# ZHENGXi-git/TC-VIML

Hardware: AMD Instinct MI355X
Metric: sliding-window solves/sec (10 kf, 200 pt, 40 line) (higher is better)
Workload: dtype f64; 1 GPU; configs[2]: synthetic 10-kf window, 200 point + 40 2D-3D line residual blocks + marginalisation prior (n=75), 50 landmarks; 8 fixed dogleg iterations + 1 MARGIN_OLD marginalisation per solve; windows_per_gpu=1024, parallelism=independent windows x1, threads_per_window=256, layout=chain

## Files before the change

### tc-viml_amd/csrc/tcv_marg.hip

```cpp
#include <hip/hip_runtime.h>

#include "tcv_factors.h"
#include "tcv_marg.h"
#include "tcv_dev.h"

namespace tcv {

__device__ __forceinline__ int pidx(int a, int b) { return a >= b ? a * (a + 1) / 2 + b : b * (b + 1) / 2 + a; }


__device__ __forceinline__ void jacobi_angle(double app, double aqq, double apq, double tiny, double &c, double &s, bool &rot) {
    c = 1.0; s = 0.0; rot = false;
    if (fabs(apq) > tiny && fabs(apq) > 1e-15 * sqrt(fabs(app) * fabs(aqq))) {
        const double tau = (aqq - app) / (2.0 * apq);
        const double t = (tau >= 0 ? 1.0 : -1.0) / (fabs(tau) + sqrt(1.0 + tau * tau));
        c = 1.0 / sqrt(1.0 + t * t);
        s = t * c;
        rot = true;
    }
}
template <int MARG_NT, typename VP>
__device__ __noinline__ int jacobi_eig(lds_d *M, VP *V, int d, int ld, lds_d *rot, lds_i *cnt, int tid, double floor_rel, gbl_d *prof = nullptr) {
    long long t_last = clock64();
#ifdef TCV_PROFILE
// ... 611 lines not shown
            for (int i = n - 2; i > rbest; i--) {
                dm = fma(-e2[i], fast_rcp(dm), dv[i] - l);
                if (fabs(dm) < pivmin) dm = -pivmin;
                Z[i * ld + k] = dm;
            }
        }
        double z = 1.0, nrm2 = 1.0;
        for (int i = rbest - 1; i >= 0; i--) {
            z = -ev[i] * fast_rcp(Z[i * ld + k]) * z;
            Z[i * ld + k] = z;
            nrm2 += z * z;
        }
        z = 1.0;
        for (int i = rbest; i + 1 < n; i++) {
            z = -ev[i] * fast_rcp(Z[(i + 1) * ld + k]) * z;
            Z[(i + 1) * ld + k] = z;
            nrm2 += z * z;
        }
        Z[rbest * ld + k] = 1.0;
        const double sc = 1.0 / sqrt(nrm2);
        for (int i = 0; i < n; i++) Z[i * ld + k] *= sc;
        resid = gbest * sc;
    }
    __syncthreads();
    EMARK(2);
    if (wave == 0) {
        const double ctol = 1e-10 * tnorm;
        int start = -1;
        for (int k = 0; k < n; k++) {
            if (!(lam[k] > 1e-8)) continue;
            if (start < 0 || lam[k] - lam[k - 1] > ctol || !(lam[k - 1] > 1e-8)) { start = k; continue; }
            for (int pass = 0; pass < 2; pass++)
                for (int j = start; j < k; j++) {
                    double dot = 0;
                    for (int r = lane; r < n; r += 64) dot += Z[r * ld + j] * Z[r * ld + k];
                    for (int o = 32; o > 0; o >>= 1) dot += __shfl_xor(dot, o);
                    for (int r = lane; r < n; r += 64) Z[r * ld + k] -= dot * Z[r * ld + j];
                    __builtin_amdgcn_fence(__ATOMIC_ACQ_REL, "wavefront");
                }
            double nn = 0;
            for (int r = lane; r < n; r += 64) { const double t = Z[r * ld + k]; nn += t * t; }
            for (int o = 32; o > 0; o >>= 1) nn += __shfl_xor(nn, o);
            const double sc = 1.0 / sqrt(nn);
            for (int r = lane; r < n; r += 64) Z[r * ld + k] *= sc;
            __builtin_amdgcn_fence(__ATOMIC_ACQ_REL, "wavefront");
        }
    }
    __syncthreads();
    EMARK(3);
    {
        int c0 = 0;
        if (!old_search) { while (c0 < n && !(lam[c0] > 1e-8)) c0++; }
        if (!(flags & 2)) eig_backtransform_wy<NT>(Hq, Z, tauv, vbuf, n, ld, tid, c0);
        else if (NT >= 512 || n - c0 <= 16 * NW) eig_backtransform<4>(Hq, Z, tauv, n, ld, tid, c0);
        else eig_backtransform<3>(Hq, Z, tauv, n, ld, tid, c0);
    }
    __syncthreads();
    EMARK(4);
    double dev = 0;
    {
        lds_d *u1 = vbuf, *u2 = pbuf;
        if (tid < n) {
            double a1 = 0, a2 = 0;
            for (int k = 0; k < n; k++) if (lam[k] > 1e-8) { const double zz = Z[tid * ld + k]; a1 += zz; a2 += (k & 1) ? -zz : zz; }
            u1[tid] = a1; u2[tid] = a2;
        }
        __syncthreads();
        if (tid < n && lam[tid] > 1e-8) {
            double t1 = 0, t2 = 0;
            for (int r2 = 0; r2 < n; r2++) { const double zz = Z[r2 * ld + tid]; t1 += zz * u1[r2]; t2 += zz * u2[r2]; }
            dev = fmax(fabs(t1 - 1.0), fabs(t2 - ((tid & 1) ? -1.0 : 1.0)));
        }
    }
    for (int o = 32; o > 0; o >>= 1) { dev = fmax(dev, __shfl_xor(dev, o)); resid = fmax(resid, __shfl_xor(resid, o)); }
    __syncthreads();
    if (lane == 0) { red[wave] = dev; red[8 + wave] = resid; }
    __syncthreads();
    dev = 0; resid = 0;
#pragma unroll
    for (int w = 0; w < NW; w++) { dev = fmax(dev, red[w]); resid = fmax(resid, red[8 + w]); }
    double sl = 0;
    for (int i = 0; i < n; i++) sl += lam[i];
    __syncthreads();
    EMARK(5);
    if (tid == 0 && dbg) { dbg[0] = dev; dbg[1] = sl; dbg[2] = trace; dbg[3] = tnorm; dbg[4] = lam[0]; dbg[5] = lam[n - 1]; }
    if (!old_search) return (dev < 1e-7) && (resid <= 1e-9 * fmax(tnorm, 1e-300) * n) && (dev == dev) && (resid == resid);
    return (dev < 1e-7) && (fabs(sl - trace) <= 1e-9 * fmax(tnorm, 1e-300) * n) && (dev == dev);
}

#ifdef TCV_PROFILE
#define MARG_MARK(id) do { const long long t_ = clock64(); if (tid == 0) out[MARG_DIAG_PHASE + (id)] += (double)(t_ - t_last); t_last = t_; } while (0)
#define MARG_SUB(id) do { const long long t_ = clock64(); if (tid == 0) out[MARG_DIAG_PROJ_SUB + (id)] += (double)(t_ - t_sub); t_sub = t_; } while (0)
#else
#define MARG_MARK(id) do { } while (0)
#define MARG_SUB(id) do { } while (0)
#endif
template <int MREG>
__device__ __noinline__ void chol_small_regs(lds_d *Mm_, lds_d *okflag_, int m_, int ldm_, int tid) {
    lds_d *Mm = opaque_lds(Mm_), *okflag = opaque_lds(okflag_);
    const int m = uni_i<2>(m_), ldm = uni_i<2>(ldm_);
    if (tid < 64) {
        const int i = min(tid, m - 1);
        double t[MREG];
#pragma unroll
        for (int c = 0; c < MREG; c++) { const double a = pin_f64(Mm[i * ldm + min(c, m - 1)]); t[c] = c < m ? a : 0.0; }
        bool ok = true;
#pragma unroll
        for (int k = 0; k < MREG; k++) {
            const double sd = lane_f64(t[k], k);
            ok = ok && (k >= m || ((sd > 0.0) && (sd < 1e300)));
            const double rs = 1.0 / sqrt((ok && k < m) ? sd : 1.0);
            const double lik = t[k] * rs;
#pragma unroll
            for (int c = k + 1; c < MREG; c++) t[c] -= lik * lane_f64(lik, c);
            if (tid < m && tid > k) Mm[tid * ldm + k] = lik;
            if (tid == k && k < m) Mm[k * ldm + k] = rs;
        }
        if (tid == 0) *okflag = ok ? 1.0 : 0.0;
    }
}
template <int MREG>
__device__ __noinline__ void fwd_small_regs(const lds_d *Mm_, const lds_d *Apk_, const lds_d *bv_, lds_d *Zl_, lds_d *rot_, int m_, int n_, int ldm_, int zs_, int tid) {
    const lds_d *Mm = opaque_lds(Mm_), *Apk = opaque_lds(Apk_), *bv = opaque_lds(bv_);
    lds_d *Zl = opaque_lds(Zl_), *rot = opaque_lds(rot_);
    const int m = uni_i<2>(m_), n = uni_i<2>(n_), ldm = uni_i<2>(ldm_), zs = uni_i<2>(zs_);
    if (tid < n + 1 + m) {
        const int j = tid, ju = tid - n - 1;
        double z[MREG];
#pragma unroll
        for (int k = 0; k < MREG; k++) {
            const int kc = min(k, m - 1);
            const double a = pin_f64(Apk[pidx(m + min(j, n - 1), kc)]), bb = pin_f64(bv[kc]);
            z[k] = k < m ? (j < n ? a : (j == n ? bb : (k == ju ? 1.0 : 0.0))) : 0.0;
        }
        double nn = 0.0;
#pragma unroll
        for (int k = 0; k < MREG; k++) {
            const int kc = min(k, m - 1);
            double l[MREG];
            const double lkk = Mm[kc * ldm + kc];
#pragma unroll
            for (int k2 = k + 1; k2 < MREG; k2++) l[k2] = Mm[min(k2, m - 1) * ldm + kc];
            z[k] *= lkk;
            nn = (k >= ju && k < m) ? fma(z[k], z[k], nn) : nn;
#pragma unroll
            for (int k2 = k + 1; k2 < MREG; k2++) z[k2] = pin_f64(z[k2] - l[k2] * z[k]);
            if (j <= n && k < m) Zl[k * zs + j] = z[k];
            __builtin_amdgcn_sched_barrier(0);
        }
        if (j > n) rot[ju] = nn;
    }
}

#ifndef TCV_MARG_WAVES
#define TCV_MARG_WAVES 2
#endif
template <int MARG_NT>
__global__ void __launch_bounds__(MARG_NT) __attribute__((disable_tail_calls)) __attribute__((amdgpu_waves_per_eu(TCV_MARG_WAVES, TCV_MARG_WAVES))) marg_kernel(MargArgs Aarg) {
    extern __shared__ __attribute__((aligned(16))) double lds_raw[];
    lds_d *lds = (lds_d *)lds_raw;
    const int tid = threadIdx.x;
    gbl_d *scr = (gbl_d *)Aarg.scratch + (size_t)blockIdx.x * MARG_SCR_STRIDE;
    for (int win = blockIdx.x; win < Aarg.nwin; win += gridDim.x) {
        typedef const __attribute__((address_space(4))) MargHdr cst_mh;
        cst_mh &H = ((cst_mh *)Aarg.hdr)[win];
        cst_i *ip = (cst_i *)Aarg.ipool + H.ibase;
        cst_d *dp = (cst_d *)Aarg.dpool + H.dbase;
        const int pos = H.pos, m = H.m, n = H.n;
        if (H.nblk == 0) {
            if (tid == 0) { ((gbl_i *)Aarg.out_status)[win] = 0; ((gbl_i *)Aarg.out_status)[Aarg.nwin + win] = 0; }
            continue;
        }
        const int npk = pos * (pos + 1) / 2;
        lds_d *Apk = lds;
        const int me = m + (m & 1), ne = n + (n & 1);
        const int r1 = max(npk, ne * (ne + 1));
        lds_d *R2 = lds + ((r1 + 1) & ~1);
        const int cb_in_r2 = (H.cb_off >= 0 && H.cb_off >= ((r1 + 1) & ~1)) ? MARG_CB_LM * H.cb_stride + 2 * MARG_CB_LM : 0;
        const int r2 = max(max((int)MARG_STAGE + cb_in_r2, me * (me + 1) + max(me * (me + 1), m * (n + 1))), (n - 2) * (n - 1) / 2 + 1);
        lds_d *bv = R2 + ((r2 + 1) & ~1);
        lds_d *x = bv + MARG_MAX_POS;
        lds_d *rot = x + ((H.nx + 7) & ~7);
        lds_d *lam = rot + 160;
        lds_d *cvec = lam + MARG_MAX_N;
        lds_d *lmacc = cvec + MARG_MAX_POS;
        lds_d *sm = lmacc + 8;
        lds_d *stage = R2;
        lds_i *cnt = (lds_i *)(rot + 158);
        gbl_d *out = (gbl_d *)Aarg.out + (size_t)win * MARG_OUT_STRIDE;
        long long t_last = clock64();
        if (tid == 0) for (int i = 0; i < 12; i++) out[MARG_DIAG_PHASE + i] = 0.0;

        cst_i *blk = ip + H.o_blk;
        for (int b = tid; b < H.nblk; b += MARG_NT) {
            const int gs = blk[b * 5], go = blk[b * 5 + 1], xs = blk[b * 5 + 4];
            for (int i = 0; i < gs; i++)
                x[go + i] = (Aarg.use_solved_state && xs >= 0 && Aarg.solve_state)
                                ? ((const gbl_d *)Aarg.solve_state)[(size_t)H.solve_window * Aarg.state_stride + xs + i]
                                : dp[H.d_x + go + i];
        }
        for (int i = tid; i < pos; i += MARG_NT) { bv[i] = 0.0; cvec[i] = 0.0; }
        if (tid < 8) lmacc[tid] = 0.0;
        cst_d *misc = dp + H.d_misc;
        const double G3[3] = {misc[0], misc[1], misc[2]};
        __syncthreads();

        MARG_MARK(0);
        bool a_zeroed = false;
        if (H.prior_n > 0) {
            const int np = H.prior_n, k0 = H.prior_k0 >= 0 ? H.prior_k0 : ((cst_win *)Aarg.solve_win)[H.solve_window].prior_k0, nr = np - k0;
            cst_d *J0 = H.prior_abs >= 0 ? (cst_d *)Aarg.solve_dpool + H.prior_abs : dp + H.d_prior, *r0 = J0 + nr * np, *x0 = r0 + nr;
            lds_d *pdx = sm, *pr = sm + 128;
            if (tid < H.prior_nblk) {
                cst_i *pb = ip + H.o_prior + tid * 4;
                const int gs = pb[2], ls = gs == 7 ? 6 : gs;
                double x0v[16], xv[16], dxv[16];
                for (int i = 0; i < 16; i++) { x0v[i] = (i < gs) ? x0[pb[3] + i] : 0.0; xv[i] = (i < gs) ? x[blk[pb[0] * 5 + 1] + i] : 0.0; }
                prior_block_dx(xv, x0v, gs, dxv);
                for (int i = 0; i < 16; i++) if (i < ls) pdx[pb[1] + i] = dxv[i];
            }
            cst_i *pcol = ip + H.o_pcol;
            const bool in_lds = np <= MARG_MAX_N && nr * np <= r1;
            lds_d *Js = Apk;
            if (in_lds) {
                for (int e = tid; e < nr * np; e += 4 * MARG_NT) {
                    double v4[4];
#pragma unroll
                    for (int k = 0; k < 4; k++) if (e + k * MARG_NT < nr * np) v4[k] = J0[e + k * MARG_NT];
#pragma unroll
                    for (int k = 0; k < 4; k++) if (e + k * MARG_NT < nr * np) Js[e + k * MARG_NT] = v4[k];
                }
            } else {
                for (int i = tid; i < npk; i += MARG_NT) Apk[i] = 0.0;
                a_zeroed = true;
            }
            __syncthreads();
            if (tid < nr) {
                double r = r0[tid];
                if (in_lds) {
                    int j = 0;
                    for (; j + 3 < np; j += 4) {
                        double a4[4], d4[4];
#pragma unroll
                        for (int u = 0; u < 4; u++) { a4[u] = Js[tid + nr * (j + u)]; d4[u] = pdx[j + u]; }
#pragma unroll
                        for (int u = 0; u < 4; u++) r += a4[u] * d4[u];
                    }
                    for (; j < np; j++) r += Js[tid + nr * j] * pdx[j];
                }
                else for (int j = 0; j < np; j++) r += J0[tid + nr * j] * pdx[j];
                pr[tid] = r;
            }
            __syncthreads();
            if (in_lds) {
                typedef double v4f64 __attribute__((ext_vector_type(4)));
                constexpr int NWV = MARG_NT / 64;
                const int nt16 = (np + 15) >> 4, lane = tid & 63, wave = tid >> 6;
                const int m16 = lane & 15, k4 = lane >> 4;
                v4f64 accs[4];
#pragma unroll
                for (int slot = 0; slot < 4; slot++) {
                    const int t = wave + slot * NWV;
                    v4f64 acc = {0.0, 0.0, 0.0, 0.0};
                    if (t < nt16 * (nt16 + 1) / 2) {
                        int ta = 0;
                        while ((ta + 1) * (ta + 2) / 2 <= t) ta++;
                        const int tb = t - ta * (ta + 1) / 2;
                        const int a = 16 * ta + m16, b = 16 * tb + m16;
                        const lds_d *ca = Js + nr * min(a, np - 1), *cb = Js + nr * min(b, np - 1);
                        for (int i0 = k0 & ~15; i0 < np; i0 += 16) {
                            double av[4], bv4[4];
#pragma unroll
                            for (int u = 0; u < 4; u++) {
                                const int i = i0 + 4 * u + k4, ic = max(0, min(i, np - 1) - k0);
                                const double xa = ca[ic], y = cb[ic];
                                av[u] = (i >= k0 && i < np && a < np) ? xa : 0.0; bv4[u] = (i >= k0 && i < np && b < np) ? y : 0.0;
                            }
#pragma unroll
                            for (int u = 0; u < 4; u++) acc = __builtin_amdgcn_mfma_f64_16x16x4f64(av[u], bv4[u], acc, 0, 0, 0);
                        }
                    }
                    accs[slot] = acc;
                }
                double s2 = 0;
                const bool mine = tid < np && pcol[min(tid, np - 1)] >= 0;
                if (mine) {
                    int i = 0;
                    for (; i + 3 < nr; i += 4) {
                        double a4[4], r4[4];
#pragma unroll
                        for (int u = 0; u < 4; u++) { a4[u] = Js[i + u + nr * tid]; r4[u] = pr[i + u]; }
#pragma unroll
                        for (int u = 0; u < 4; u++) s2 += a4[u] * r4[u];
                    }
                    for (; i < nr; i++) s2 += Js[i + nr * tid] * pr[i];
                }
                __syncthreads();
                for (int i = tid; i < npk; i += MARG_NT) Apk[i] = 0.0;
                a_zeroed = true;
                __syncthreads();
#pragma unroll
                for (int slot = 0; slot < 4; slot++) {
                    const int t = wave + slot * NWV;
                    if (t < nt16 * (nt16 + 1) / 2) {
                        int ta = 0;
                        while ((ta + 1) * (ta + 2) / 2 <= t) ta++;
                        const int tb = t - ta * (ta + 1) / 2;
#pragma unroll
                        for (int i = 0; i < 4; i++) {
                            const int ga = 16 * ta + 4 * i + k4, gb = 16 * tb + m16;
                            if (ga < np && gb <= ga) { const int ia = pcol[ga], ib = pcol[gb]; if (ia >= 0 && ib >= 0) Apk[pidx(ia, ib)] += accs[slot][i]; }
                        }
                    }
                }
                if (mine) bv[pcol[tid]] += s2;
            } else {
                for (int e = tid; e < np * np; e += MARG_NT) {
                    const int a = e / np, b = e - a * np;
                    if (b > a) continue;
                    const int ia = pcol[a], ib = pcol[b];
                    if (ia < 0 || ib < 0) continue;
                    double s0 = 0;
                    for (int i = 0; i < nr; i++) s0 += J0[i + nr * a] * J0[i + nr * b];
                    Apk[pidx(ia, ib)] += s0;
                }
                if (tid < np && pcol[tid] >= 0) {
                    double s2 = 0;
                    for (int i = 0; i < nr; i++) s2 += J0[i + nr * tid] * pr[i];
                    bv[pcol[tid]] += s2;
                }
            }
            __syncthreads();
        }
        if (!a_zeroed) {
            for (int i = tid; i < npk; i += MARG_NT) Apk[i] = 0.0;
            __syncthreads();
        }
        MARG_MARK(1);
        cst_d *imu0 = H.imu_abs >= 0 ? (cst_d *)Aarg.solve_dpool + H.imu_abs : dp + H.d_imu;
        for (int f = 0; f < H.n_imu; f++) {
            cst_i *b = ip + H.o_imu + f * 4;
            lds_d *S = stage + 1500;
            const bool s_given = Aarg.solve_sqrt != nullptr && H.sqrt_src >= 0 && H.n_imu == 1;
            if (s_given) { for (int i = tid; i < 225; i += MARG_NT) S[i] = ((const gbl_d *)Aarg.solve_sqrt)[(size_t)H.solve_window * 225 + i]; }
            else if (tid < 16) (void)imu_sqrt_info_group(imu0 + f * IMU_CONST + IMU_COV, S, stage + 512, stage + 512 + 225, tid);
            constexpr int RW0 = MARG_NT >= 320 ? 1 : 0, RLANE = MARG_NT >= 320 ? 0 : 32;
            if ((tid & 63) == RLANE && (tid >> 6) >= RW0 && (tid >> 6) < RW0 + 4) {
                double cst[62];
#pragma unroll
                for (int i = 0; i < 62; i++) cst[i] = imu0[f * IMU_CONST + i];
                imu_raw_part((tid >> 6) - RW0, CGEN(x + blk[b[0] * 5 + 1]), CGEN(x + blk[b[1] * 5 + 1]), CGEN(x + blk[b[2] * 5 + 1]),
                             CGEN(x + blk[b[3] * 5 + 1]), cst, G3, GEN(stage), IMU_STRIDE_J, true);
            }
            __syncthreads();
            if (tid < 31) {
                lds_d *rec = stage + tid;
                double v[15];
                for (int r = 0; r < 15; r++) v[r] = rec[r * IMU_STRIDE_J];
                for (int r = 0; r < 15; r++) {
                    double a = 0;
                    for (int s2 = r; s2 < 15; s2++) a += S[r * 15 + s2] * v[s2];
                    rec[r * IMU_STRIDE_J] = a;
                }
            }
            __syncthreads();
            const int colc[4] = {0, 6, 15, 21};
            for (int e = tid; e < 30 * 31; e += MARG_NT) {
                const int ca = e / 31, cb = e - ca * 31;
                if (cb < 30 && cb > ca) continue;
                int sa = 0, sb = 0;
                while (sa < 3 && ca >= colc[sa + 1]) sa++;
                const int la = blk[b[sa] * 5 + 2];
                if (la < 0) continue;
                const int ia = la + ca - colc[sa];
                double s = 0;
                for (int r = 0; r < 15; r++) s += stage[r * IMU_STRIDE_J + ca] * stage[r * IMU_STRIDE_J + cb];
                if (cb == 30) { bv[ia] += s; continue; }
                while (sb < 3 && cb >= colc[sb + 1]) sb++;
                const int lb = blk[b[sb] * 5 + 2];
                if (lb < 0) continue;
                Apk[pidx(ia, lb + cb - colc[sb])] += s;
            }
            __syncthreads();
        }
        MARG_MARK(2);
        const bool with_td = H.td_blk >= 0;
        const int prs = with_td ? 21 : (int)PROJ_STRIDE, prr = with_td ? 43 : (int)PROJ_REC;
        const int njc = with_td ? 20 : 19;
        const bool cb_path = H.block_mode && H.cb_off >= 0;
#ifdef TCV_PROFILE
        long long t_sub = clock64();
        if (tid == 0) for (int i = 0; i < 4; i++) out[MARG_DIAG_PROJ_SUB + i] = 0.0;
#endif
        MARG_SUB(0);
        typedef __attribute__((address_space(3))) unsigned char lds_b;
        lds_i *gtab = (lds_i *)sm, *ncls = gtab + 336;
        lds_b *listS = (lds_b *)(gtab + 340), *listJ = listS + 96, *listL = listJ + 104;
        if (cb_path) {
            if (tid < 3) ncls[tid] = 0;
            __syncthreads();
            const int ntri = 19 * 20 / 2;
            if (tid < ntri + 19) {
                int ca, cb;
                if (tid < ntri) { ca = (int)((sqrt(8.0 * (double)tid + 1.0) - 1.0) * 0.5); while ((ca + 1) * (ca + 2) / 2 <= tid) ca++; while (ca * (ca + 1) / 2 > tid) ca--; cb = tid - ca * (ca + 1) / 2; }
                else { ca = tid - ntri; cb = 19; }
                const int ga = ca < 18 ? ca / 6 : 3, gb = cb < 18 ? cb / 6 : 3;
                const int cls = ca == 18 ? 2 : ((ga == 1 || (cb < 18 && gb == 1)) ? 1 : 0);
                const int at = atomicAdd((int *)(ncls + cls), 1);
                (cls == 0 ? listS : (cls == 1 ? listJ : listL))[at] = (unsigned char)tid;
            }
            __syncthreads();
        }
        for (int pc = 0; cb_path && pc < H.n_pchunk; pc++) {
            cst_i *pch = ip + H.o_pchunk + pc * 4;
            const int f0 = pch[0], fn = pch[1];
            lds_d *Cb = lds + H.cb_off, *hl = Cb + MARG_CB_LM * H.cb_stride, *glv = hl + MARG_CB_LM;
            lds_i *ftab = (lds_i *)cvec;
            const int cbs = H.cb_stride;
            for (int i = tid; i < MARG_CB_LM * cbs + 2 * MARG_CB_LM; i += MARG_NT) Cb[i] = 0.0;
            {
                cst_i *gsrc = ip + H.o_pgrp + pch[3];
                const int glen = gsrc[3];
                for (int i = tid; i < glen; i += MARG_NT) gtab[i] = gsrc[i];
            }
            if (tid < fn) {
                cst_i *pf = ip + H.o_proj + (f0 + tid) * 4;
                lds_d *rec = stage + tid * prr;
                double r[2], pts[6];
#pragma unroll
                for (int i = 0; i < 6; i++) pts[i] = dp[H.d_proj + (f0 + tid) * 6 + i];
                proj_eval(CGEN(x + blk[pf[0] * 5 + 1]), CGEN(x + blk[pf[1] * 5 + 1]), CGEN(x + blk[pf[2] * 5 + 1]), x[blk[pf[3] * 5 + 1]],
                          pts, misc[3], r, GEN(rec), PROJ_STRIDE);
                (void)loss_correct2(r, GEN(rec), 19, PROJ_STRIDE, misc[4]);
                rec[19] = r[0]; rec[PROJ_STRIDE + 19] = r[1];
                unsigned wq = 0;
#pragma unroll
                for (int k = 0; k < 4; k++) wq |= (unsigned)((blk[pf[k] * 5 + 2] + 1) & 255) << (8 * k);
                ftab[2 * tid] = (int)wq;
                ftab[2 * tid + 1] = ip[H.o_plm + f0 + tid] + 1;
            }
            __syncthreads();
            MARG_SUB(1);
            {
                const int nfr = gtab[0], nlg = gtab[1], uniform = gtab[2];
                cst_i *dummy_plm = ip + H.o_plm + f0; (void)dummy_plm;
                const lds_i *fr = gtab + 4, *lg = fr + 2 * nfr, *fl = lg + 2 * nlg;
                const int nS = ncls[0], nJ = ncls[1], nL = ncls[2];
                const int secS = (nS + 63) & ~63, secJ = (nfr * nJ + 63) & ~63, secL = nlg * nL;
                const int o_bv = (int)(bv - lds), o_cb = (int)(Cb - lds), o_hl = (int)(hl - lds), o_gl = (int)(glv - lds);
                for (int task = tid; task < secS + secJ + secL; task += MARG_NT) {
                    int t, kind, g0 = 0, cnt = fn;
                    if (task < secS) { if (task >= nS) continue; kind = 0; t = listS[task]; }
                    else if (task < secS + secJ) {
                        const int q = task - secS;
                        if (q >= nfr * nJ) continue;
                        const int sfr = q / nJ;
                        kind = 1; t = listJ[q - sfr * nJ]; g0 = fr[2 * sfr]; cnt = fr[2 * sfr + 1];
                    } else {
                        const int q = task - secS - secJ, sl = q / nL;
                        kind = 2; t = listL[q - sl * nL]; g0 = lg[2 * sl]; cnt = lg[2 * sl + 1];
                    }
                    const int ntri = 19 * 20 / 2;
                    int ca, cb;
                    if (t < ntri) { ca = (int)((sqrt(8.0 * (double)t + 1.0) - 1.0) * 0.5); while ((ca + 1) * (ca + 2) / 2 <= t) ca++; while (ca * (ca + 1) / 2 > t) ca--; cb = t - ca * (ca + 1) / 2; }
                    else { ca = t - ntri; cb = 19; }
                    const int ga = ca < 18 ? ca / 6 : 3, oa = ca < 18 ? ca % 6 : 0;
                    const int gb = cb < 18 ? cb / 6 : 3, ob = cb < 18 ? cb % 6 : 0;
                    const int rb = cb == 19 ? 19 : cb;
                    auto dest = [&](int f) -> int {
                        const unsigned w = (unsigned)ftab[2 * f];
                        const int lml = ftab[2 * f + 1] - 1;
                        const int la = (int)((w >> (8 * ga)) & 255u) - 1, lb = (int)((w >> (8 * gb)) & 255u) - 1;
                        if (ca == 18 && lml >= 0) {
                            if (cb < 18) return lb >= 0 ? o_cb + lml * cbs + lb + ob : -1;
                            return (cb == 18 ? o_hl : o_gl) + lml;
                        }
                        if (la >= 0 && (cb == 19 || lb >= 0)) return cb == 19 ? o_bv + la + oa : pidx(la + oa, lb + ob);
                        return -1;
                    };
                    if (uniform && !(kind == 2 && cb < 18 && gb == 1)) {
                        const int d = dest(kind == 1 ? fl[g0] : g0);
                        if (d < 0) continue;
                        double accv = lds[d];
                        int k = 0;
                        for (; k + 3 < cnt; k += 4) {
                            double s4[4];
#pragma unroll
                            for (int u = 0; u < 4; u++) {
                                const int f = kind == 1 ? fl[g0 + k + u] : g0 + k + u;
                                const lds_d *rec = stage + f * prr;
                                s4[u] = rec[ca] * rec[rb] + rec[prs + ca] * rec[prs + rb];
                            }
#pragma unroll
                            for (int u = 0; u < 4; u++) accv += s4[u];
                        }
                        for (; k < cnt; k++) {
                            const int f = kind == 1 ? fl[g0 + k] : g0 + k;
                            const lds_d *rec = stage + f * prr;
                            accv += rec[ca] * rec[rb] + rec[prs + ca] * rec[prs + rb];
                        }
                        lds[d] = accv;
                        continue;
                    }
                    int prev = -1;
                    double accv = 0.0;
                    for (int k = 0; k < cnt; k++) {
                        const int f = kind == 1 ? fl[g0 + k] : g0 + k;
                        const lds_d *rec = stage + f * prr;
                        const double sv = rec[ca] * rec[rb] + rec[prs + ca] * rec[prs + rb];
                        const int d = dest(f);
                        if (d < 0) continue;
                        if (d != prev) {
                            if (prev >= 0) lds[prev] = accv;
                            accv = lds[d];
                            prev = d;
                        }
                        accv += sv;
                    }
                    if (prev >= 0) lds[prev] = accv;
                }
            }
            __syncthreads();
            MARG_SUB(2);
            {
                typedef double v4f64 __attribute__((ext_vector_type(4)));
                constexpr int NWV = MARG_NT / 64;
                const int lane = tid & 63, wave = tid >> 6, col = lane & 15, row0 = lane >> 4;
                const int nt16 = (pos + 15) >> 4;
                double ih[4];
#pragma unroll
                for (int kk = 0; kk < 4; kk++) { const double h = hl[4 * kk + row0]; ih[kk] = h > 1e-8 ? 1.0 / h : 0.0; }
                for (int t = wave; t < nt16 * (nt16 + 1) / 2; t += NWV) {
                    int I = 0;
                    while ((I + 1) * (I + 2) / 2 <= t) I++;
                    const int J = t - I * (I + 1) / 2;
                    double av[4], bw[4];
// ... 64 lines not shown
                        const int la = ga == 0 ? l0 : (ga == 1 ? l1 : (ga == 2 ? l2 : (ga == 3 ? l3 : ltd)));
                        const int lb = gb == 0 ? l0 : (gb == 1 ? l1 : (gb == 2 ? l2 : (gb == 3 ? l3 : ltd)));
                        const lds_d *rec = stage + f * prr;
                        const double sv = rec[ra] * rec[rb] + rec[prs + ra] * rec[prs + rb];
                        const int d = (la < 0 || (cb != njc && lb < 0)) ? -1 : (cb == njc ? MARG_MAX_POS * MARG_MAX_POS + la + oa : pidx(la + oa, lb + ob));
                        if (d < 0) continue;
                        if (d != prev) {
                            if (prev >= 0) { if (prev >= MARG_MAX_POS * MARG_MAX_POS) bv[prev - MARG_MAX_POS * MARG_MAX_POS] = accv; else Apk[prev] = accv; }
                            accv = d >= MARG_MAX_POS * MARG_MAX_POS ? bv[d - MARG_MAX_POS * MARG_MAX_POS] : Apk[d];
                            prev = d;
                        }
                        accv += sv;
                    }
                    if (prev >= 0) { if (prev >= MARG_MAX_POS * MARG_MAX_POS) bv[prev - MARG_MAX_POS * MARG_MAX_POS] = accv; else Apk[prev] = accv; }
                }
                __syncthreads();
                continue;
            }
            for (int f = 0; f < fn; f++) {
                cst_i *pf = ip + H.o_proj + (f0 + f) * 4;
                const lds_d *rec = stage + f * prr;
                for (int e = tid; e < njc * (njc + 1); e += MARG_NT) {
                    const int ca = e / (njc + 1), cb = e - ca * (njc + 1);
                    if (cb < njc && cb > ca) continue;
                    const int ba = ca < 18 ? pf[ca / 6] : (ca == 18 ? pf[3] : H.td_blk), oa = ca < 18 ? ca % 6 : 0;
                    const int ra = ca == 19 ? 20 : ca, rb = cb == njc ? 19 : (cb == 19 ? 20 : cb);
                    const int la = blk[ba * 5 + 2];
                    const double s = rec[ra] * rec[rb] + rec[prs + ra] * rec[prs + rb];
                    if (H.block_mode && ca == 18) {
                        if (cb == 18) lmacc[0] += s;
                        else if (cb == njc) lmacc[1] += s;
                        else { const int bb = cb < 18 ? pf[cb / 6] : H.td_blk, lb = blk[bb * 5 + 2]; if (lb >= 0) cvec[lb + (cb < 18 ? cb % 6 : 0)] += s; }
                        continue;
                    }
                    if (H.block_mode && ca == 19 && cb == 18) {
                        if (la >= 0) cvec[la] += s;
                        continue;
                    }
                    if (la < 0) continue;
                    const int ia = la + oa;
                    if (cb == njc) { bv[ia] += s; continue; }
                    const int bb = cb < 18 ? pf[cb / 6] : (cb == 18 ? pf[3] : H.td_blk);
                    const int lb = blk[bb * 5 + 2];
                    if (lb < 0) continue;
                    Apk[pidx(ia, lb + (cb < 18 ? cb % 6 : 0))] += s;
                }
                __syncthreads();
                if (H.block_mode && ip[H.o_plast + f0 + f]) {
                    const double d = lmacc[0], g = lmacc[1], invd = d > 1e-8 ? 1.0 / d : 0.0;
                    for (int e = tid; e < pos * pos; e += MARG_NT) {
                        const int i = e / pos, j = e - i * pos;
                        if (j > i) continue;
                        const double ci = cvec[i], cj = cvec[j];
                        if (ci != 0.0 && cj != 0.0) Apk[pidx(i, j)] -= ci * cj * invd;
                    }
                    if (tid < pos) bv[tid] -= cvec[tid] * g * invd;
                    __syncthreads();
                    for (int i = tid; i < pos; i += MARG_NT) cvec[i] = 0.0;
                    if (tid == 0) { lmacc[0] = 0.0; lmacc[1] = 0.0; }
                    __syncthreads();
                }
            }
        }
        MARG_MARK(3);
        const int ldm = me + 1;
        lds_d *Mm = R2, *Vm = R2 + me * ldm;
        lds_d *Zl = Vm;
        const int zs = n + 1;
        for (int i = tid; i < m * m; i += MARG_NT) { const int r = i / m, c = i - r * m; Mm[r * ldm + c] = Apk[pidx(r, c)]; }
        __syncthreads();
        bool chol = Aarg.eig_mm == 0;
        constexpr int MREG = 24;
        if (chol && m <= MREG) {
            chol_small_regs<MREG>(Mm, lmacc + 2, m, ldm, tid);
            MARG_MARK(9);
            __syncthreads();
            MARG_MARK(10);
            chol = lmacc[2] != 0.0;
        } else
        if (chol) {
            if (tid < 64) {
                const int i = min(tid, m - 1);
                bool ok = true;
                for (int k = 0; k < m; k++) {
                    double sv = Mm[i * ldm + k], sd = Mm[k * ldm + k];
                    int p2 = 0;
                    for (; p2 + 3 < k; p2 += 4) {
                        double lk[4], li[4];
#pragma unroll
                        for (int u = 0; u < 4; u++) { lk[u] = Mm[k * ldm + p2 + u]; li[u] = Mm[i * ldm + p2 + u]; }
#pragma unroll
                        for (int u = 0; u < 4; u++) { sv -= li[u] * lk[u]; sd -= lk[u] * lk[u]; }
                    }
                    for (; p2 < k; p2++) { const double lk = Mm[k * ldm + p2]; sv -= Mm[i * ldm + p2] * lk; sd -= lk * lk; }
                    ok = ok && (sd > 0.0) && (sd < 1e300);
                    const double rs = 1.0 / sqrt(ok ? sd : 1.0);
                    __builtin_amdgcn_fence(__ATOMIC_ACQ_REL, "wavefront");
                    if (tid < m && tid > k) Mm[tid * ldm + k] = sv * rs;
                    if (tid == k) Mm[k * ldm + k] = rs;
                    __builtin_amdgcn_fence(__ATOMIC_ACQ_REL, "wavefront");
                }
                if (tid == 0) lmacc[2] = ok ? 1.0 : 0.0;
            }
            __syncthreads();
            chol = lmacc[2] != 0.0;
        }
        if (chol && m <= MREG) {
            fwd_small_regs<MREG>(Mm, Apk, bv, Zl, rot, m, n, ldm, zs, tid);
            MARG_MARK(11);
            __syncthreads();
            double tr = 0, trs = 0;
            for (int j = 0; j < m; j++) { tr += rot[j]; trs += rot[j] * Apk[pidx(j, j)]; }
            chol = tr < 1e8;
            if (tid == 0) { out[MARG_DIAG_AMM_TRACE] = tr; out[MARG_DIAG_AMM_TRACE + 1] = trs; }
        } else
        if (chol) {
            if (tid < n + 1) {
                const int j = tid;
                for (int k = 0; k < m; k++) {
                    double sv = j < n ? Apk[pidx(m + j, k)] : bv[k];
                    int p2 = 0;
                    for (; p2 + 3 < k; p2 += 4) {
                        double lk[4], zz[4];
#pragma unroll
                        for (int u = 0; u < 4; u++) { lk[u] = Mm[k * ldm + p2 + u]; zz[u] = Zl[(p2 + u) * zs + j]; }
#pragma unroll
                        for (int u = 0; u < 4; u++) sv -= lk[u] * zz[u];
                    }
                    for (; p2 < k; p2++) sv -= Mm[k * ldm + p2] * Zl[p2 * zs + j];
                    Zl[k * zs + j] = sv * Mm[k * ldm + k];
                }
            } else if (tid < n + 1 + m) {
                const int j = tid - n - 1;
                double y = Mm[j * ldm + j], nn = y * y;
                lds_d *yr = Mm + j * ldm;
                for (int k = j + 1; k < m; k++) {
                    double sv = -Mm[k * ldm + j] * y;
                    for (int p2 = j + 1; p2 < k; p2++) sv -= Mm[k * ldm + p2] * yr[p2];
                    sv *= Mm[k * ldm + k];
                    yr[k] = sv;
                    nn += sv * sv;
                }
                rot[j] = nn;
            }
            __syncthreads();
            double tr = 0, trs = 0;
            for (int j = 0; j < m; j++) { tr += rot[j]; trs += rot[j] * Apk[pidx(j, j)]; }
            chol = tr < 1e8;
            if (tid == 0) { out[MARG_DIAG_AMM_TRACE] = tr; out[MARG_DIAG_AMM_TRACE + 1] = trs; }
        }
        int sweeps1 = 0;
        const int ldn = ne + 1;
        lds_d *As = Apk, *V2 = Apk;
        double keepA[ (MARG_MAX_N * MARG_MAX_N + MARG_NT - 1) / MARG_NT ];
        bool keep_sym = false;
        double bprime = 0;
        gbl_d *Z = scr + MARG_SCR_Z, *zb = scr + MARG_SCR_PR;
        if (chol) {
            MARG_MARK(4);
            MARG_MARK(5);
            int q = 0;
            keep_sym = true;
            for (int e = tid; e < ((n + 1) >> 1) * (n + 1); e += MARG_NT, q++) {
                const int R = e / (n + 1), Cc = e - R * (n + 1);
                const int i = (Cc <= R) ? R : n - 1 - R, j = (Cc <= R) ? Cc : Cc - R - 1;
                double sv = Apk[pidx(m + i, m + j)];
                int k = 0;
                for (; k + 3 < m; k += 4) {
                    double za[4], zb4[4];
#pragma unroll
                    for (int u = 0; u < 4; u++) { za[u] = Zl[(k + u) * zs + i]; zb4[u] = Zl[(k + u) * zs + j]; }
#pragma unroll
                    for (int u = 0; u < 4; u++) sv -= za[u] * zb4[u];
                }
                for (; k < m; k++) sv -= Zl[k * zs + i] * Zl[k * zs + j];
                keepA[q] = sv;
            }
            if (tid < n) {
                bprime = bv[m + tid];
                for (int k = 0; k < m; k++) bprime -= Zl[k * zs + tid] * Zl[k * zs + n];
            }
        } else {
            if (Aarg.eig_mm == 0) {
                __syncthreads();
                for (int i = tid; i < m * m; i += MARG_NT) { const int r = i / m, c2 = i - r * m; Mm[r * ldm + c2] = Apk[pidx(r, c2)]; }
                __syncthreads();
            }
            sweeps1 = jacobi_eig<MARG_NT, lds_d>(Mm, Vm, m, ldm, rot, cnt, tid, 0.0);
            MARG_MARK(4);
            if (tid < m) { const double l = Mm[tid * ldm + tid]; lam[tid] = l > 1e-8 ? sqrt(1.0 / l) : 0.0; }
            __syncthreads();
            for (int e = tid; e < m * n; e += MARG_NT) {
                const int k = e / n, j = e - k * n;
                double sv = 0;
                for (int p2 = 0; p2 < m; p2++) sv += Vm[p2 * ldm + k] * Apk[pidx(m + j, p2)];
                Z[k * n + j] = lam[k] * sv;
            }
            if (tid < m) {
                double sv = 0;
                for (int p2 = 0; p2 < m; p2++) sv += Vm[p2 * ldm + tid] * bv[p2];
                zb[tid] = lam[tid] * sv;
            }
            __syncthreads();
            MARG_MARK(5);
            int q = 0;
            for (int e = tid; e < n * n; e += MARG_NT, q++) {
                const int i = e / n, j = e - i * n;
                double sv = Apk[pidx(m + i, m + j)];
                for (int k = 0; k < m; k++) sv -= Z[k * n + i] * Z[k * n + j];
                keepA[q] = sv;
            }
            if (tid < n) {
                bprime = bv[m + tid];
                for (int k = 0; k < m; k++) bprime -= Z[k * n + tid] * zb[k];
            }
        }
        __syncthreads();
        {
            int q = 0;
            if (keep_sym) {
                for (int e = tid; e < ((n + 1) >> 1) * (n + 1); e += MARG_NT, q++) {
                    const int R = e / (n + 1), Cc = e - R * (n + 1);
                    const int i = (Cc <= R) ? R : n - 1 - R, j = (Cc <= R) ? Cc : Cc - R - 1;
                    As[i * ldn + j] = keepA[q]; As[j * ldn + i] = keepA[q];
                    out[MARG_OUT_AS + i * n + j] = keepA[q]; out[MARG_OUT_AS + j * n + i] = keepA[q];
                }
            } else
            for (int e = tid; e < n * n; e += MARG_NT, q++) {
                const int i = e / n, j = e - i * n;
                As[i * ldn + j] = keepA[q];
                out[MARG_OUT_AS + i * n + j] = keepA[q];
            }
        }
        if (tid < n) { bv[tid] = bprime; out[MARG_OUT_BS + tid] = bprime; }
        __syncthreads();
        MARG_MARK(6);
        int sweeps2 = 0;
        {
            const bool ok = sym_eig_tridiag<MARG_NT>(As, R2, sm, rot, n, ldn, tid, out + MARG_DIAG_EIG_CHECK, Aarg.eig_flags);
            if (ok) {
                if (tid < n) lam[tid] = rot[tid];
            } else {
                gbl_d *Vg = scr + MARG_SCR_V;
                for (int e = tid; e < n * n; e += MARG_NT) { const int i2 = e / n, j2 = e - i2 * n; As[i2 * ldn + j2] = out[MARG_OUT_AS + i2 * n + j2]; }
                __syncthreads();
                sweeps2 = 100 + jacobi_eig<MARG_NT, gbl_d>(As, Vg, n, ldn, rot, cnt, tid, 2.3e-16, out + MARG_DIAG_PHASE + 9);
                if (tid < n) lam[tid] = As[tid * ldn + tid];
                __syncthreads();
                for (int e = tid; e < n * n; e += MARG_NT) { const int i2 = e / n, j2 = e - i2 * n; V2[i2 * ldn + j2] = Vg[i2 * ldn + j2]; }
            }
        }
        MARG_MARK(7);
        __syncthreads();
        bool bad = false;
        if (tid < n) {
            const double l = lam[tid];
            int rank = 0;
            for (int j = 0; j < n; j++) rank += (lam[j] < l || (lam[j] == l && j < tid)) ? 1 : 0;
            const double S = l > 1e-8 ? l : 0.0, Sinv = l > 1e-8 ? 1.0 / l : 0.0;
            const double ss = sqrt(S), si = sqrt(Sinv);
            double rb = 0;
            for (int j = 0; j < n; j++) {
                const double v = V2[j * ldn + tid];
                out[MARG_OUT_J0 + rank + n * j] = ss * v;
                rb += v * bv[j];
            }
            out[MARG_OUT_R0 + rank] = si * rb;
            if (!(si * rb == si * rb) || !(l == l)) bad = true;
        }
        if (tid < 64) {
            const bool z0 = tid < n && !(lam[tid] > 1e-8), z1 = tid + 64 < n && !(lam[tid + 64] > 1e-8);
            int k0 = __popcll(__ballot(z0)) + __popcll(__ballot(z1));
            if (k0 >= n) k0 = n > 0 ? n - 1 : 0;
            if (tid == 0) ((gbl_i *)Aarg.out_status)[Aarg.nwin + win] = k0;
        }
        for (int i = tid; i < H.nx; i += MARG_NT) out[MARG_OUT_X + i] = x[i];
        MARG_MARK(8);
        if (tid == 0) ((gbl_i *)Aarg.out_status)[win] = (sweeps1 >= 24 || sweeps2 == 124) ? 1 : (sweeps2 >= 100 ? 2 : 0);
        if (tid == 0) { out[MARG_DIAG_SWEEPS_MM] = sweeps1; out[MARG_DIAG_SWEEPS_RR] = sweeps2; }
        __syncthreads();
        if (bad) ((gbl_i *)Aarg.out_status)[Aarg.nwin + win] = -1;
    }
}

template <int NT> static int launch_marg_nt(const MargArgs &a, int grid, size_t lds_bytes, hipStream_t st) {
    hipError_t e = hipFuncSetAttribute((const void *)marg_kernel<NT>, hipFuncAttributeMaxDynamicSharedMemorySize, (int)lds_bytes);
    if (e != hipSuccess) return hip_fail(e, "hipFuncSetAttribute(marg)");
    hipLaunchKernelGGL(marg_kernel<NT>, dim3(grid), dim3(NT), lds_bytes, st, a);
    if ((e = hipGetLastError()) != hipSuccess) return hip_fail(e, "marg kernel launch");
    return TCV_OK;
}

__global__ void __launch_bounds__(256) prior_splice_kernel(const PriorSplice *jobs, double *dpool, WinHdr *wins) {
    const PriorSplice &J = jobs[blockIdx.x];
    const int tid = threadIdx.x;
    int k0 = J.k0;
    if (J.kind == 0 && J.k0_src) {
        k0 = max(0, min(J.n - 1, *J.k0_src));
        if (tid == 0) wins[J.win].prior_k0 = k0;
    }
    const int n = J.n, nr = n - k0;
    const double *src = J.src;
    double *dst = dpool + J.dst;
    if (J.kind == 1) {
        for (int i = tid; i < 287; i += 256) {
            double v;
            if (i < 17) v = src[i];
            else if (i < 62) {
                const int q = i - 17, blk = q / 9, e = q - 9 * blk, r = e / 3, c = e - 3 * r;
                const int r0 = (blk < 2) ? 0 : (blk == 2 ? 3 : 6), c0 = (blk == 0 || blk == 3) ? 9 : 12;
                v = src[17 + (r0 + r) * 15 + c0 + c];
            } else v = src[242 + (i - 62)];
            dst[i] = v;
        }
        return;
    }
    for (int e = tid; e < nr * n; e += 256) { const int j = e / nr, i = e - j * nr; dst[e] = src[MARG_OUT_J0 + (size_t)n * j + k0 + i]; }
    for (int i = tid; i < nr; i += 256) dst[nr * n + i] = src[MARG_OUT_R0 + k0 + i];
    int xo = nr * n + nr;
    for (int k = 0; k < J.nblk; k++) {
        if (tid < J.size[k]) dst[xo + tid] = src[MARG_OUT_X + J.goff[k] + tid];
        xo += J.size[k];
    }
}
int launch_prior_splice(const PriorSplice *d_jobs, int njobs, double *d_dpool, void *d_win_headers, hipStream_t st) {
    if (njobs <= 0) return TCV_OK;
    hipLaunchKernelGGL(prior_splice_kernel, dim3(njobs), dim3(256), 0, st, d_jobs, d_dpool, (WinHdr *)d_win_headers);
    const hipError_t e = hipGetLastError();
    if (e != hipSuccess) return hip_fail(e, "prior splice kernel launch");
    return TCV_OK;
}

}

int tcv_launch_marg(const tcv::MargArgs *args, int grid, int nt, size_t lds_bytes, hipStream_t st) {
    return nt == tcv::MARG_NT_PAIR ? tcv::launch_marg_nt<tcv::MARG_NT_PAIR>(*args, grid, lds_bytes, st)
                                   : tcv::launch_marg_nt<tcv::MARG_NT_WIDE>(*args, grid, lds_bytes, st);
}
```

Measured before the change: 230,300 solves/s.

## Use f64 MFMA for marginalisation Schur complement and IMU info products

Replaces the scalar per-thread Schur complement accumulation (A_rr - Z^T Z) with 16x16x4 f64 MFMA tiles over the lower triangle, held in registers until write-back. The IMU sqrt-information multiply and the J^T J accumulation are also recast as small MFMA tiles. The eigenvector output loop is restructured so each thread writes coalesced elements using a rank table in LDS, and dot products are unrolled by 4. These are aimed at scalar FMA and uncoalesced store costs in the marginalisation kernel, at the price of padding waste for small n and extra register pressure.

```diff
diff --git a/tc-viml_amd/csrc/tcv_marg.hip b/tc-viml_amd/csrc/tcv_marg.hip
--- a/tc-viml_amd/csrc/tcv_marg.hip
+++ b/tc-viml_amd/csrc/tcv_marg.hip
@@ -787,6 +787,38 @@
     }
 }
 
+#ifndef TCV_MP
+#define TCV_MP 7
+#endif
+typedef double mg_v4 __attribute__((ext_vector_type(4)));
+template <int MARG_NT> struct SchurTiles { enum { NWV = MARG_NT / 64, NT16 = (MARG_MAX_N + 15) / 16, SLOTS = (NT16 * (NT16 + 1) / 2 + NWV - 1) / NWV }; };
+__device__ __forceinline__ void tri_tile(int t, int &ta, int &tb) { ta = 0; while ((ta + 1) * (ta + 2) / 2 <= t) ta++; tb = t - ta * (ta + 1) / 2; }
+template <int MARG_NT, class ZP>
+__device__ __forceinline__ void schur_tiles(mg_v4 (&accs)[SchurTiles<MARG_NT>::SLOTS], const lds_d *Apk, const ZP *Zp, int zs, int m, int n, int tid) {
+    typedef SchurTiles<MARG_NT> ST;
+    if (n <= 0) return;
+    const int nt16 = (n + 15) >> 4, lane = tid & 63, wave = tid >> 6, m16 = lane & 15, k4 = lane >> 4;
+    int ca[ST::SLOTS], cb[ST::SLOTS];
+#pragma unroll
+    for (int slot = 0; slot < ST::SLOTS; slot++) {
+        const int t = wave + slot * ST::NWV;
+        int ta, tb;
+        tri_tile(t < nt16 * (nt16 + 1) / 2 ? t : 0, ta, tb);
+        ca[slot] = min(16 * ta + m16, n - 1); cb[slot] = min(16 * tb + m16, n - 1);
+#pragma unroll
+        for (int i = 0; i < 4; i++) accs[slot][i] = Apk[pidx(m + min(16 * ta + 4 * i + k4, n - 1), m + cb[slot])];
+    }
+    for (int kq = 0; kq < m; kq += 4) {
+        const int k = kq + k4, kc = min(k, m - 1);
+        double za[ST::SLOTS], zb[ST::SLOTS];
+#pragma unroll
+        for (int slot = 0; slot < ST::SLOTS; slot++) { za[slot] = Zp[kc * zs + ca[slot]]; zb[slot] = Zp[kc * zs + cb[slot]]; }
+#pragma unroll
+        for (int slot = 0; slot < ST::SLOTS; slot++)
+            accs[slot] = __builtin_amdgcn_mfma_f64_16x16x4f64(-(k < m ? za[slot] : 0.0), k < m ? zb[slot] : 0.0, accs[slot], 0, 0, 0);
+    }
+}
+
 #ifndef TCV_MARG_WAVES
 #define TCV_MARG_WAVES 2
 #endif
@@ -987,6 +1019,61 @@
                 imu_raw_part((tid >> 6) - RW0, CGEN(x + blk[b[0] * 5 + 1]), CGEN(x + blk[b[1] * 5 + 1]), CGEN(x + blk[b[2] * 5 + 1]),
                              CGEN(x + blk[b[3] * 5 + 1]), cst, G3, GEN(stage), IMU_STRIDE_J, true);
             }
+#if TCV_MP & 2
+            lds_i *icol = (lds_i *)sm;
+            if (tid < 32) {
+                const int colc[4] = {0, 6, 15, 21};
+                const int c = min(tid, 29);
+                int sa = 0;
+                while (sa < 3 && c >= colc[sa + 1]) sa++;
+                const int la = blk[b[sa] * 5 + 2];
+                icol[tid] = (tid < 30 && la >= 0) ? la + c - colc[sa] : -1;
+            }
+            __syncthreads();
+            {
+                const int lane = tid & 63, wave = tid >> 6, i16 = lane & 15, k4 = lane >> 4;
+                if (wave < 2) {
+                    const int col = 16 * wave + i16;
+                    double sa[4], bb[4];
+#pragma unroll
+                    for (int kk = 0; kk < 4; kk++) {
+                        const int k = 4 * kk + k4;
+                        const double ts = S[min(i16, 14) * 15 + min(k, 14)], tv = stage[min(k, 14) * IMU_STRIDE_J + min(col, 30)];
+                        sa[kk] = (i16 < 15 && k < 15 && k >= i16) ? ts : 0.0; bb[kk] = (k < 15 && col < 31) ? tv : 0.0;
+                    }
+                    mg_v4 acc = {0.0, 0.0, 0.0, 0.0};
+#pragma unroll
+                    for (int kk = 0; kk < 4; kk++) acc = __builtin_amdgcn_mfma_f64_16x16x4f64(sa[kk], bb[kk], acc, 0, 0, 0);
+#pragma unroll
+                    for (int i = 0; i < 4; i++) { const int row = k4 + 4 * i; if (row < 15 && col < 31) stage[row * IMU_STRIDE_J + col] = acc[i]; }
+                }
+                __syncthreads();
+                if (wave < 3) {
+                    const int I = wave >= 1 ? 1 : 0, J = wave == 2 ? 1 : 0;
+                    const int ca = 16 * I + i16, cb = 16 * J + i16;
+                    double oa[4], ob[4];
+#pragma unroll
+                    for (int kk = 0; kk < 4; kk++) {
+                        const int k = 4 * kk + k4;
+                        const double ta = stage[min(k, 14) * IMU_STRIDE_J + min(ca, 30)], tb = stage[min(k, 14) * IMU_STRIDE_J + min(cb, 30)];
+                        oa[kk] = (k < 15 && ca < 31) ? ta : 0.0; ob[kk] = (k < 15 && cb < 31) ? tb : 0.0;
+                    }
+                    mg_v4 acc = {0.0, 0.0, 0.0, 0.0};
+#pragma unroll
+                    for (int kk = 0; kk < 4; kk++) acc = __builtin_amdgcn_mfma_f64_16x16x4f64(oa[kk], ob[kk], acc, 0, 0, 0);
+                    const int ib = icol[cb];
+#pragma unroll
+                    for (int i = 0; i < 4; i++) {
+                        const int ra = 16 * I + 4 * i + k4;
+                        if (ra > 30 || cb >= 30 || cb > ra || ib < 0) continue;
+                        if (ra == 30) { bv[ib] += acc[i]; continue; }
+                        const int ia = icol[ra];
+                        if (ia >= 0) Apk[pidx(ia, ib)] += acc[i];
+                    }
+                }
+            }
+            __syncthreads();
+#else
             __syncthreads();
             if (tid < 31) {
                 lds_d *rec = stage + tid;
@@ -1017,6 +1104,7 @@
                 Apk[pidx(ia, lb + cb - colc[sb])] += s;
             }
             __syncthreads();
+#endif
         }
         MARG_MARK(2);
         const bool with_td = H.td_blk >= 0;
@@ -1387,13 +1475,20 @@
         int sweeps1 = 0;
         const int ldn = ne + 1;
         lds_d *As = Apk, *V2 = Apk;
+#if TCV_MP & 1
+        mg_v4 keepT[SchurTiles<MARG_NT>::SLOTS];
+#else
         double keepA[ (MARG_MAX_N * MARG_MAX_N + MARG_NT - 1) / MARG_NT ];
         bool keep_sym = false;
+#endif
         double bprime = 0;
         gbl_d *Z = scr + MARG_SCR_Z, *zb = scr + MARG_SCR_PR;
         if (chol) {
             MARG_MARK(4);
             MARG_MARK(5);
+#if TCV_MP & 1
+            schur_tiles<MARG_NT>(keepT, Apk, Zl, zs, m, n, tid);
+#else
             int q = 0;
             keep_sym = true;
             for (int e = tid; e < ((n + 1) >> 1) * (n + 1); e += MARG_NT, q++) {
@@ -1411,9 +1506,22 @@
                 for (; k < m; k++) sv -= Zl[k * zs + i] * Zl[k * zs + j];
                 keepA[q] = sv;
             }
+#endif
             if (tid < n) {
                 bprime = bv[m + tid];
+#if TCV_MP & 1
+                int k = 0;
+                for (; k + 3 < m; k += 4) {
+                    double za[4], zb4[4];
+#pragma unroll
+                    for (int u = 0; u < 4; u++) { za[u] = Zl[(k + u) * zs + tid]; zb4[u] = Zl[(k + u) * zs + n]; }
+#pragma unroll
+                    for (int u = 0; u < 4; u++) bprime -= za[u] * zb4[u];
+                }
+                for (; k < m; k++) bprime -= Zl[k * zs + tid] * Zl[k * zs + n];
+#else
                 for (int k = 0; k < m; k++) bprime -= Zl[k * zs + tid] * Zl[k * zs + n];
+#endif
             }
         } else {
             if (Aarg.eig_mm == 0) {
@@ -1438,6 +1546,9 @@
             }
             __syncthreads();
             MARG_MARK(5);
+#if TCV_MP & 1
+            schur_tiles<MARG_NT>(keepT, Apk, Z, n, m, n, tid);
+#else
             int q = 0;
             for (int e = tid; e < n * n; e += MARG_NT, q++) {
                 const int i = e / n, j = e - i * n;
@@ -1445,12 +1556,36 @@
                 for (int k = 0; k < m; k++) sv -= Z[k * n + i] * Z[k * n + j];
                 keepA[q] = sv;
             }
+#endif
             if (tid < n) {
                 bprime = bv[m + tid];
                 for (int k = 0; k < m; k++) bprime -= Z[k * n + tid] * zb[k];
             }
         }
         __syncthreads();
+#if TCV_MP & 1
+        {
+            typedef SchurTiles<MARG_NT> ST;
+            const int nt16 = (n + 15) >> 4, lane = tid & 63, wave = tid >> 6, m16 = lane & 15, k4 = lane >> 4;
+#pragma unroll
+            for (int slot = 0; slot < ST::SLOTS; slot++) {
+                const int t = wave + slot * ST::NWV;
+                if (t < nt16 * (nt16 + 1) / 2) {
+                    int ta, tb;
+                    tri_tile(t, ta, tb);
+#pragma unroll
+                    for (int i = 0; i < 4; i++) {
+                        const int ga = 16 * ta + 4 * i + k4, gb = 16 * tb + m16;
+                        if (ga < n && gb <= ga) {
+                            const double v = keepT[slot][i];
+                            As[ga * ldn + gb] = v; As[gb * ldn + ga] = v;
+                            out[MARG_OUT_AS + ga * n + gb] = v; out[MARG_OUT_AS + gb * n + ga] = v;
+                        }
+                    }
+                }
+            }
+        }
+#else
         {
             int q = 0;
             if (keep_sym) {
@@ -1467,6 +1602,7 @@
                 out[MARG_OUT_AS + i * n + j] = keepA[q];
             }
         }
+#endif
         if (tid < n) { bv[tid] = bprime; out[MARG_OUT_BS + tid] = bprime; }
         __syncthreads();
         MARG_MARK(6);
@@ -1488,6 +1624,52 @@
         MARG_MARK(7);
         __syncthreads();
         bool bad = false;
+#if TCV_MP & 4
+        lds_d *srank = rot;
+        lds_i *crank = (lds_i *)(rot + MARG_MAX_N);
+        int rank = 0;
+        double si = 0.0;
+        if (tid < n) {
+            const double l = lam[tid];
+            for (int j0 = 0; j0 < n; j0 += 8) {
+                double lj[8];
+#pragma unroll
+                for (int u = 0; u < 8; u++) lj[u] = lam[min(j0 + u, n - 1)];
+#pragma unroll
+                for (int u = 0; u < 8; u++) rank += (j0 + u < n && (lj[u] < l || (lj[u] == l && j0 + u < tid))) ? 1 : 0;
+            }
+            const double S = l > 1e-8 ? l : 0.0, Sinv = l > 1e-8 ? 1.0 / l : 0.0;
+            srank[rank] = sqrt(S); crank[rank] = tid;
+            si = sqrt(Sinv);
+        }
+        __syncthreads();
+        for (int o0 = tid; o0 < n * n; o0 += 4 * MARG_NT) {
+            double s4[4], v4[4];
+#pragma unroll
+            for (int u = 0; u < 4; u++) {
+                const unsigned o = (unsigned)min(o0 + u * MARG_NT, n * n - 1), j = o / (unsigned)n, rk = o - j * (unsigned)n;
+                const int c = min(max(crank[rk], 0), n - 1);
+                s4[u] = srank[rk]; v4[u] = V2[j * ldn + c];
+            }
+#pragma unroll
+            for (int u = 0; u < 4; u++) if (o0 + u * MARG_NT < n * n) out[MARG_OUT_J0 + o0 + u * MARG_NT] = s4[u] * v4[u];
+        }
+        if (tid < n) {
+            const double l = lam[tid];
+            double rb = 0;
+            int j = 0;
+            for (; j + 3 < n; j += 4) {
+                double v4[4], b4[4];
+#pragma unroll
+                for (int u = 0; u < 4; u++) { v4[u] = V2[(j + u) * ldn + tid]; b4[u] = bv[j + u]; }
+#pragma unroll
+                for (int u = 0; u < 4; u++) rb += v4[u] * b4[u];
+            }
+            for (; j < n; j++) rb += V2[j * ldn + tid] * bv[j];
+            out[MARG_OUT_R0 + rank] = si * rb;
+            if (!(si * rb == si * rb) || !(l == l)) bad = true;
+        }
+#else
         if (tid < n) {
             const double l = lam[tid];
             int rank = 0;
@@ -1503,6 +1685,7 @@
             out[MARG_OUT_R0 + rank] = si * rb;
             if (!(si * rb == si * rb) || !(l == l)) bad = true;
         }
+#endif
         if (tid < 64) {
             const bool z0 = tid < n && !(lam[tid] > 1e-8), z1 = tid + 64 < n && !(lam[tid + 64] > 1e-8);
             int k0 = __popcll(__ballot(z0)) + __popcll(__ballot(z1));
```

Measured after the change: 231,100 solves/s (median of 6 runs). About the same (+0.3%).
